# krm01/Snappy.jl

Hardware: AMD Instinct MI355X
Metric: GB/s compressed+decompressed (batched blocks) at 1/2/4/8 GPUs; % HBM peak (higher is better)
Workload: dtype u8; 1 GPU; configs 2+3: 10000 x 64 KiB text blocks per GPU, fast-mode compress + uncompress round trip per step; blocks_per_gpu=10000, block_bytes=65536, parallelism=dp1 (blocks sharded per rank, RCCL size all-gather)

## Files before the change

### snappy.jl_amd/csrc/sm_dec_walk.h

```cpp
#pragma once
#include "sm_device.h"

namespace sm {

typedef uint16_t __attribute__((aligned(1))) du16u;
typedef uint32_t __attribute__((aligned(1))) du32u;
typedef uint64_t __attribute__((aligned(1))) du64u;

constexpr uint32_t kMaxBatchLit = 200;
constexpr int kWalkLevels = 5;
constexpr int kJtRow = 256;
constexpr int kJt = kWalkLevels * kJtRow / 2;
__device__ inline uint32_t load_word(const uint8_t* __restrict__ in, uint32_t N, uint32_t p) {
  if (p + 3 < N && (((uintptr_t)(in + p)) & 3) == 0) return *reinterpret_cast<const uint32_t*>(in + p);
  uint32_t v = 0;
#pragma unroll
  for (int k = 0; k < 4; ++k) v |= (p + k < N ? (uint32_t)in[p + k] : 0u) << (8 * k);
  return v;
}

__device__ inline uint64_t load8z(const uint8_t* __restrict__ in, uint32_t N, uint32_t p) {
  return (uint64_t)load_word(in, N, p) | ((uint64_t)load_word(in, N, p + 4) << 32);
}

__device__ inline uint32_t pack_sizes(uint32_t cur, uint32_t nxt) {
  const uint32_t K = cur & 0x03030303u, H = (cur >> 2) & 0x3f3f3f3fu;
  const uint32_t csz = __builtin_amdgcn_perm(0u, 0x05030200u, K);
  const uint32_t ml = __builtin_amdgcn_perm(0u, 0x000000ffu, K);
  uint32_t sz = (csz & ~ml) | ((H + 0x02020202u) & ml);
  const uint32_t h60 = (H + 0x44444444u) & 0x80808080u & ml;
  if (h60) {
    const uint32_t hm = h60 | (h60 - (h60 >> 7));
    const uint32_t b = __builtin_amdgcn_alignbyte(nxt, cur, 1);
    const uint32_t e = cur ^ 0xf0f0f0f0u;
    const uint32_t ne = (((e & 0x7f7f7f7fu) + 0x7f7f7f7fu) | e) & 0x80808080u;
    const uint32_t bb = (((b >> 1) & 0x7f7f7f7fu) + 0x1c1c1c1cu) & 0x80808080u;
    const uint32_t st = ne | bb;
    const uint32_t sm = st | (st - (st >> 7));
    const uint32_t v = (b | sm) + (0x03030303u & ~sm);
    sz = (sz & ~hm) | (v & hm);
  }
  return sz;
}

__device__ inline bool walk_stop_literal(uint32_t c, uint64_t lit) {
  return (c & 3) == 0 && ((c >> 2) >= 61 || lit > kMaxBatchLit);
}

__device__ inline uint32_t walk_window(uint64_t cw, uint32_t rlim, uint16_t* jt16, uint32_t lane, uint32_t& cpos,
                                       uint32_t& csz, uint32_t& sizes) {
  uint8_t* const jt = reinterpret_cast<uint8_t*>(jt16);
  rlim = min(rlim, 255u);
  sizes = pack_sizes((uint32_t)cw, (uint32_t)(cw >> 32));
  auto rd = [&](int k, uint32_t x) -> uint32_t { return jt[k * kJtRow + x]; };
  auto row = [&](int k, const uint32_t (&J)[4]) {
    *reinterpret_cast<uint32_t*>(jt + k * kJtRow + 4 * lane) = J[0] | (J[1] << 8) | (J[2] << 16) | (J[3] << 24);
  };
  uint32_t J[4];
#pragma unroll
  for (int j = 0; j < 4; ++j) {
    const uint32_t p = 4 * lane + j;
    const uint32_t sz = (sizes >> (8 * j)) & 0xff;
    J[j] = sz == 255 ? p : min(p + sz, 255u);
  }
  row(0, J);
  uint32_t c = 0;
#pragma unroll
  for (int k = 1; k < kWalkLevels; ++k) {
    __atomic_signal_fence(__ATOMIC_SEQ_CST);
    const uint32_t t = rd(k - 1, c);
#pragma unroll
    for (int j = 0; j < 4; ++j) J[j] = rd(k - 1, J[j]);
    c = ((lane >> (k - 1)) & 1u) ? t : c;
    row(k, J);
  }
  __atomic_signal_fence(__ATOMIC_SEQ_CST);
  {
    const uint32_t t = rd(kWalkLevels - 1, c);
    c = ((lane >> (kWalkLevels - 1)) & 1u) ? t : c;
  }
  if (lane >= 32) {
    c = rd(kWalkLevels - 1, c);
    c = rd(kWalkLevels - 1, c);
  }
  const uint32_t szw = __shfl(sizes, (c >> 2) & 63u, 64);
  const uint32_t sz = (szw >> (8 * (c & 3))) & 0xffu;
  cpos = c;
  csz = sz;
  __atomic_signal_fence(__ATOMIC_SEQ_CST);
  return (uint32_t)__builtin_popcountll(ballot(c < rlim && sz != 255));
}

__device__ inline void stage_bytes(uint8_t* buf, const uint8_t* __restrict__ in, uint32_t N, uint32_t s, uint32_t len,
                                   uint32_t lane) {
  constexpr int kU = 6;
  uint32_t* dst = reinterpret_cast<uint32_t*>(buf);
  const uint32_t nw = (len + 3) / 4;
  if (N == 0) {
    for (uint32_t k = lane; k < nw; k += kWave) dst[k] = 0;
    return;
  }
  const uint32_t mis = (uint32_t)((uintptr_t)(in + s) & 3u);
  const uint32_t* src = reinterpret_cast<const uint32_t*>(in + s - mis);
  const int64_t klast = ((intptr_t)((uintptr_t)(in + N - 1) & ~(uintptr_t)3) - (intptr_t)src) / 4;
  for (uint32_t k0 = lane; k0 < nw; k0 += kU * kWave) {
    uint32_t w[kU];
#pragma unroll
    for (int u = 0; u < kU; ++u) {
      const int64_t k = k0 + u * kWave;
      w[u] = __builtin_amdgcn_alignbyte(src[min(k + 1, klast)], src[min(k, klast)], mis);
    }
#pragma unroll
    for (int u = 0; u < kU; ++u) {
      const uint64_t b = (uint64_t)s + 4 * (k0 + u * kWave);
      const uint64_t v = b < N ? (uint64_t)N - b : 0u;
      w[u] &= v >= 4 ? 0xffffffffu : (uint32_t)((1ull << (8 * v)) - 1);
    }
#pragma unroll
    for (int u = 0; u < kU; ++u)
      if (k0 + u * kWave < nw) dst[k0 + u * kWave] = w[u];
  }
}

__device__ inline Tag tag_at(const uint8_t* buf, uint32_t rel) { return decode_tag8(lds_ld64(buf, rel)); }

__device__ inline uint32_t window_tags(const uint8_t* buf, uint32_t rel0, uint32_t rlim, uint16_t* jt, uint32_t lane,
                                       uint32_t& rel, uint32_t& next, uint32_t& outb, uint32_t& excl) {
  uint32_t cpos, csz, sizes;
  const uint32_t ntok = walk_window(lds_ld64(buf, rel0 + 4 * lane), rlim, jt, lane, cpos, csz, sizes);
  const bool mine = lane < ntok;
  const uint32_t c = buf[rel0 + (mine ? cpos : 0u)];
  outb = !mine ? 0u : window_out_bytes(c, csz);
  excl = scan_dpp(outb) - outb;
  rel = rel0 + cpos;
  next = rel + csz;
  return ntok;
}

__device__ inline int32_t parse_header(const uint8_t* in, uint32_t N, uint32_t lane, uint32_t& size, uint32_t& ip) {
  const uint32_t hb = (lane < 5 && lane < N) ? in[lane] : 0;
  return smc::parse_varint32([&](uint32_t i) { return readlane(hb, i); }, N, size, ip);
}

}
```

### snappy.jl_amd/csrc/sm_decompress.hip

```cpp
#include "sm_dec_walk.h"
#include "sm_internal.h"

namespace sm {

constexpr uint32_t kRing = 1024;
constexpr uint32_t kRingMirror = 96;


__device__ inline void ring_put(uint8_t* ring, uint32_t base, uint32_t word, uint32_t lane) {
  uint32_t r = base & (kRing - 1);
  reinterpret_cast<uint32_t*>(ring + r)[lane] = word;
  if (r == 0 && lane < kRingMirror / 4) reinterpret_cast<uint32_t*>(ring + kRing)[lane] = word;
}

__device__ inline uint64_t ring_get8(const uint8_t* ring, uint32_t pos) { return lds_ld64(ring, pos & (kRing - 1)); }

__device__ inline void ring_fill(const uint8_t* __restrict__ in, uint32_t N, uint32_t wb, uint8_t* ring, uint32_t& pre1,
                                 uint32_t& pre2, uint32_t lane) {
  uint32_t w[5];
  if ((((uintptr_t)(in + wb)) & 3) == 0 && wb + 1280 <= N) {
    const uint32_t* s = reinterpret_cast<const uint32_t*>(in + wb) + lane;
#pragma unroll
    for (int i = 0; i < 5; ++i) w[i] = s[64 * i];
  } else {
#pragma unroll
    for (int i = 0; i < 5; ++i) w[i] = load_word(in, N, wb + 256 * i + 4 * lane);
  }
  ring_put(ring, wb, w[0], lane);
  ring_put(ring, wb + 256, w[1], lane);
  ring_put(ring, wb + 512, w[2], lane);
  pre1 = w[3];
  pre2 = w[4];
}

#ifndef SM_DEC_WIN
#define SM_DEC_WIN 2560
#endif
constexpr uint32_t kWin = SM_DEC_WIN;
#ifndef SM_DEC_BOUT
#define SM_DEC_BOUT 512
#endif
constexpr uint32_t kBatchOut = SM_DEC_BOUT;
#ifndef SM_DEC_KEEP
#define SM_DEC_KEEP 480
#endif
constexpr uint32_t kKeep = SM_DEC_KEEP;
constexpr uint32_t kWinPad = 16;
static_assert(kKeep + 15 + kBatchOut + 32 <= kWin && kKeep >= 80 && kWin % 16 == 0, "window bounds");
static_assert(kKeep + 15 <= 16 * kWave, "win_shift moves at most one 16-byte unit per lane");

typedef __attribute__((address_space(3))) uint32_t lds_u32;

__device__ inline uint4 lds_get16(uint32_t a, uint32_t k) {
  const lds_u32* w = (const lds_u32*)(size_t)((a & ~3u) + k);
  const uint32_t w0 = w[0], w1 = w[1], w2 = w[2], w3 = w[3], w4 = w[4];
  return make_uint4(__builtin_amdgcn_alignbyte(w1, w0, a), __builtin_amdgcn_alignbyte(w2, w1, a),
                    __builtin_amdgcn_alignbyte(w3, w2, a), __builtin_amdgcn_alignbyte(w4, w3, a));
}

__device__ inline uint4 trim16(uint4 v, uint32_t len) {
  uint32_t l8 = len << 3;
  asm("" : "+v"(l8));
  uint64_t mlo, mhi;
  asm("v_lshrrev_b64 %0, %1, -1" : "=v"(mlo) : "v"(64 - min(l8, 64u)));
  asm("v_lshrrev_b64 %0, %1, -1" : "=v"(mhi) : "v"(128 - l8));
  const bool hi = len > 8;
  return make_uint4(v.x & (uint32_t)mlo, v.y & (uint32_t)(mlo >> 32), hi ? v.z & (uint32_t)mhi : 0u,
                    hi ? v.w & (uint32_t)(mhi >> 32) : 0u);
}

__device__ inline void lds_or16(uint32_t a, uint32_t k, uint4 v) {
  const uint32_t wa = ((a - 1u) & ~3u) + k, t = 0u - a;
  const uint32_t u0 = __builtin_amdgcn_alignbyte(v.x, 0u, t);
  const uint32_t u1 = __builtin_amdgcn_alignbyte(v.y, v.x, t);
  const uint32_t u2 = __builtin_amdgcn_alignbyte(v.z, v.y, t);
  const uint32_t u3 = __builtin_amdgcn_alignbyte(v.w, v.z, t);
  const uint32_t u4 = __builtin_amdgcn_alignbyte(0u, v.w, t);
  asm volatile("ds_or_b32 %0, %1\nds_or_b32 %0, %2 offset:4\nds_or_b32 %0, %3 offset:8\nds_or_b32 %0, %4 offset:12\n"
               "ds_or_b32 %0, %5 offset:16"
               : : "v"(wa), "v"(u0), "v"(u1), "v"(u2), "v"(u3), "v"(u4) : "memory");
}

__device__ inline void win_init(uint8_t* win, uint32_t lane) {
  for (uint32_t u = lane; u < kWin / 16; u += kWave) reinterpret_cast<uint4*>(win)[u] = make_uint4(0, 0, 0, 0);
}

__device__ inline void win_shift(uint8_t* win, uint32_t& wbase, uint32_t op, uint32_t lane) {
  const uint32_t nb = (op - kKeep) & ~15u;
  const uint32_t d = nb - wbase, n = (op - nb + 15) >> 4;
  uint4* w = reinterpret_cast<uint4*>(win);
  uint4 v = make_uint4(0, 0, 0, 0);
  if (lane < n) v = w[(d >> 4) + lane];
  __atomic_signal_fence(__ATOMIC_SEQ_CST);
  for (uint32_t u = lane; u < kWin / 16; u += kWave) w[u] = u < n ? v : make_uint4(0, 0, 0, 0);
  wbase = nb;
}

__device__ inline void win_flush(uint8_t* out, const uint8_t* win, uint32_t wbase, uint32_t from, uint32_t to,
                                 uint32_t lane) {
  if (to <= from) return;
  const uint32_t h = min((16u - (from & 15u)) & 15u, to - from);
  if (lane < h) out[from + lane] = win[from + lane - wbase];
  from += h;
  const uint32_t nb = (to - from) >> 4;
  for (uint32_t k = lane; k < nb; k += kWave) {
    const uint32_t x = from + 16 * k;
    const uint4 v = *reinterpret_cast<const uint4*>(win + (x - wbase));
    *reinterpret_cast<du64u*>(out + x) = ((uint64_t)v.y << 32) | v.x;
    *reinterpret_cast<du64u*>(out + x + 8) = ((uint64_t)v.w << 32) | v.z;
  }
  from += nb << 4;
  if (lane < to - from) out[from + lane] = win[from + lane - wbase];
}

template <uint32_t kLit = 4, bool kWhole = false>
__device__ int32_t decode_stream_batch(const uint8_t* __restrict__ in, uint32_t N, uint32_t ip, uint32_t ip_end,
                                       uint32_t size, uint8_t* out, uint32_t op0, uint32_t frag_lo, uint8_t* ring,
                                       uint16_t* jt, uint8_t* win, uint32_t lane, uint32_t& op_end,
                                       uint32_t op_lim = 0xffffffffu) {
  if (kWhole) {
    ip_end = N;
    frag_lo = 0;
    op_lim = 0xffffffffu;
  }
  uint32_t wb = ip & ~255u;
  uint32_t pre1, pre2;
  ring_fill(in, N, wb, ring, pre1, pre2, lane);
  bool issue_pre2 = false;
  uint32_t op = op0, flushed = op0;
  const uint32_t wlo = op0 & ~15u;
  uint32_t wbase = wlo;
  win_init(win, lane);
  const uint32_t winA = lds_addr(win), ringA = lds_addr(ring);
  const bool in_al = (((uintptr_t)in) & 3) == 0;
  const int64_t Nm1 = min((int64_t)N - 1, (int64_t)ip_end);

  uint32_t guard = N + 1;
  const bool narrow = N < 0x80000000u && size <= 0xffff0000u;
  while ((int64_t)ip < Nm1 && (kWhole || op < op_lim)) {
    if (__builtin_expect(--guard == 0, 0)) return kErrDevice;
    if (ip >= wb + 256) {
      if (__builtin_expect(ip < wb + 512, 1)) {
        ring_put(ring, wb + 768, pre1, lane);
        pre1 = pre2;
        wb += 256;
        issue_pre2 = true;
      } else {
        wb = ip & ~255u;
        ring_fill(in, N, wb, ring, pre1, pre2, lane);
        issue_pre2 = false;
      }
    }
    const uint32_t wlim = (int64_t)(ip + 256) < Nm1 ? ip + 256 : (uint32_t)Nm1;
    uint32_t cpos, csz, sizes;
    const uint32_t ntok = walk_window(ring_get8(ring, ip + 4 * lane), wlim - ip, jt, lane, cpos, csz, sizes);
    uint32_t tpos = 0, ipw = ip, tnext = 0;
    bool big = false;
    if (__builtin_expect(ntok != 0, 1)) {
      tpos = ip + cpos;
      tnext = cpos + csz;
      ipw = ip + readlane(tnext, ntok - 1);
    }
    if (ipw < wlim) {
      const uint32_t rel = ipw - ip;
      big = ((readlane(sizes, rel >> 2) >> ((rel & 3) * 8)) & 0xff) == 255;
    }

    if (__builtin_expect(ntok != 0, 1)) {
      const bool mine = lane < ntok;
      const uint64_t hv = ring_get8(ring, mine ? tpos : wb);
      const uint32_t c = (uint32_t)hv & 0xff;
      const uint32_t kind = c & 3, hi = c >> 2;
      const bool iscopy = kind != 0, k1 = kind == 1;
      const uint32_t len = k1 ? 4 + (hi & 7) : hi + 1;
      const uint32_t offhi = k1 ? (c << 3) & 0x700u : 0u;
      const uint32_t tl = (c + 16) >> 8;
      const uint32_t tr_raw = (uint32_t)(hv >> 8);
      uint64_t hm;
      asm("v_lshlrev_b64 %0, %1, -1" : "=v"(hm) : "v"(8 * csz - 8));
      const uint32_t offset = offhi + (tr_raw & ~(uint32_t)hm);
      const uint32_t litlen = csz - 1 - tl;
      const uint32_t olen = mine ? (iscopy ? len : litlen) : 0u;
      const uint32_t incl = scan_dpp(olen);
      const uint32_t opt = op + incl - olen;
      const uint32_t lsrc = tpos + 1 + tl;
      const uint64_t minem = ntok == 64 ? ~0ull : ((1ull << ntok) - 1);
      const uint64_t copya = ballot(iscopy) & minem;

      const uint32_t X_all = readlane(incl, ntok - 1);
      const bool clean = narrow && op <= size && op + X_all <= size && ipw <= N;
      uint64_t badm = ballot(opt <= offset - 1u);
      if (!kWhole) badm |= ballot(opt - offset < frag_lo);
      if (__builtin_expect(!clean || (badm & copya) != 0, 0)) {
        const int64_t avail_out = (int64_t)size - (int64_t)opt;
        const int64_t avail_in = (int64_t)N - (int64_t)lsrc;
        const bool e_off = (int64_t)opt <= (int64_t)(uint32_t)(offset - 1u);
        const bool e_cross = !kWhole && opt - offset < frag_lo;
        const bool e_len = !((len <= 16) & (offset >= 8) & (avail_out >= 16)) & (avail_out < (int64_t)len);
        const bool e_lit = (avail_out < (int64_t)litlen) | (avail_in < (int64_t)litlen);
        const int32_t ec = e_off ? kErrCopyOffset : (e_cross ? kErrCross : (e_len ? kErrCopyLength : kOk));
        const int32_t err = !mine ? kOk : (iscopy ? ec : (e_lit ? kErrLiteral : kOk));
        const uint64_t em = ballot(err != kOk);
        if (em != 0) return (int32_t)readlane((uint32_t)err, ctz64(em));
      }
      uint32_t nt = ntok;
      if (__builtin_expect(X_all > kBatchOut || (!kWhole && readlane(opt, ntok - 1) >= op_lim), 0)) {
        nt = (uint32_t)__builtin_popcountll(ballot(mine && incl <= kBatchOut && (kWhole || opt < op_lim)));
        ipw = ip + readlane(tnext, nt - 1);
        big = false;
      }
      const uint32_t X = readlane(incl, nt - 1);

      if (op - wbase + X + 32 > kWin) win_shift(win, wbase, op, lane);
      const uint32_t O0 = op;
      const uint32_t slo = opt - offset;
      const uint32_t shi = slo + min(len, offset);
      const uint64_t all = nt == 64 ? ~0ull : ((1ull << nt) - 1);
      const uint64_t copym = copya & all;
      const uint64_t longm = ballot(litlen > 64) & ~copym & all;
      const uint64_t gm = ballot(slo < wbase) & copym;
      const bool gsrc = inverse_ballot(gm);
      uint64_t done = longm | ~all;
      if (gm) __threadfence_block();

      uint64_t lm = longm;
      while (lm) {
        const uint32_t t = ctz64(lm);
        lm &= lm - 1;
        const uint32_t o = readlane(opt, t), sr = readlane(lsrc, t), L = readlane(litlen, t);
        const uint32_t k = 16 * lane;
        if (k < L) lds_or16(winA + (o - wbase) + k, 0, trim16(lds_get16(ringA + ((sr + k) & (kRing - 1)), 0), min(16u, L - k)));
      }

      if (__builtin_expect(done != ~0ull, 1)) {
        const uint64_t rm = ~done & (~copym | (ballot(shi <= O0) & ballot(offset >= 16)));
        const uint32_t L = iscopy ? len : litlen;
        const uint32_t sa = iscopy ? winA + (slo - wbase) : ringA + (lsrc & (kRing - 1));
        const uint32_t da = winA + (opt - wbase);
        const uint8_t* gs = out + slo;
#pragma unroll
        for (uint32_t base = 0; base < 64; base += 16) {
          const uint64_t am = rm & ballot(L > base);
          if (!am) break;
          if (inverse_ballot(am)) {
            uint4 v;
            if (gsrc) {
              const du64u* g = reinterpret_cast<const du64u*>(gs + base);
              const uint64_t a = g[0], b = g[1];
              v = make_uint4((uint32_t)a, (uint32_t)(a >> 32), (uint32_t)b, (uint32_t)(b >> 32));
            } else {
              v = lds_get16(sa, base);
            }
            lds_or16(da, base, trim16(v, min(L - base, 16u)));
          }
        }
        done |= rm;
      }
      __atomic_signal_fence(__ATOMIC_SEQ_CST);
      uint64_t rest = ~done;
      while (rest) {
        const uint32_t t = ctz64(rest);
        rest &= rest - 1;
        const uint32_t o = readlane(opt, t), sl = readlane(slo, t), L = readlane(len, t), off = readlane(offset, t);
        if (lane < L) {
          uint32_t k = lane;
          if (k >= off) {
            const uint32_t q = (uint32_t)(((float)k + 0.5f) * __builtin_amdgcn_rcpf((float)off));
            k -= q * off;
          }
          win[o + lane - wbase] = win[sl + k - wbase];
        }
        __atomic_signal_fence(__ATOMIC_SEQ_CST);
      }
      op += X;
      if (!kWhole && __builtin_expect(op > op_lim, 0)) return kErrCross;
      win_flush(out, win, wbase, flushed, op & ~15u, lane);
      flushed = max(flushed, op & ~15u);
      ip = ipw;
    }
    if (issue_pre2) {
      pre2 = (in_al && wb + 1280 <= N) ? reinterpret_cast<const uint32_t*>(in + wb + 1024)[lane]
                                       : load_word(in, N, wb + 1024 + 4 * lane);
      issue_pre2 = false;
    }

    if (__builtin_expect(big && (kWhole || op < op_lim), 0)) {
      const uint64_t hv = ring_get8(ring, ip);
      const Tag t = with_trailer(tag_head(uniform((uint32_t)hv & 0xff)), uniform((uint32_t)(hv >> 8)));
      const uint32_t litlen = t.literal_len();
      const uint32_t lsrc = ip + 1 + t.taglen;
      const int64_t avail_out = (int64_t)size - (int64_t)op;
      const int64_t avail_in = (int64_t)N - (int64_t)lsrc;
      if (avail_out < (int64_t)litlen || avail_in < (int64_t)litlen) return kErrLiteral;
      if (!kWhole && (uint64_t)op + litlen > op_lim) return kErrCross;
      if (litlen <= kMaxBatchLit) {
        if (op - wbase + litlen + 32 > kWin) win_shift(win, wbase, op, lane);
        const uint32_t k = 16 * lane;
        if (k < litlen)
          lds_or16(winA + (op - wbase) + k, 0, trim16(lds_get16(ringA + ((lsrc + k) & (kRing - 1)), 0), min(16u, litlen - k)));
        __atomic_signal_fence(__ATOMIC_SEQ_CST);
        op += litlen;
        win_flush(out, win, wbase, flushed, op & ~15u, lane);
        flushed = max(flushed, op & ~15u);
        ip = lsrc + litlen;
        continue;
      }
      win_flush(out, win, wbase, flushed, op, lane);
      const uint8_t* s = in + lsrc;
      uint32_t head = (uint32_t)((16 - ((uintptr_t)s & 15)) & 15);
      if (head > litlen) head = litlen;
      if (lane < head) out[op + lane] = s[lane];
      const uint4* s16 = reinterpret_cast<const uint4*>(s + head);
      const uint32_t n16 = (litlen - head) >> 4;
      uint8_t* d = out + op + head;
      uint32_t k = lane;
      for (; k + (kLit - 1) * kWave < n16; k += kLit * kWave) {
        uint4 v[kLit];
#pragma unroll
        for (uint32_t j = 0; j < kLit; ++j) v[j] = s16[k + j * kWave];
#pragma unroll
        for (uint32_t j = 0; j < kLit; ++j) {
          *reinterpret_cast<du64u*>(d + 16 * (k + j * kWave)) = ((uint64_t)v[j].y << 32) | v[j].x;
          *reinterpret_cast<du64u*>(d + 16 * (k + j * kWave) + 8) = ((uint64_t)v[j].w << 32) | v[j].z;
        }
      }
      for (; k < n16; k += kWave) {
        uint4 v0 = s16[k];
        *reinterpret_cast<du64u*>(d + 16 * k) = ((uint64_t)v0.y << 32) | v0.x;
        *reinterpret_cast<du64u*>(d + 16 * k + 8) = ((uint64_t)v0.w << 32) | v0.z;
      }
      const uint32_t done16 = head + (n16 << 4);
      if (lane < litlen - done16) out[op + done16 + lane] = s[done16 + lane];
      const uint32_t opn = op + litlen;
      const uint32_t nb = (opn - min(opn - wlo, kKeep)) & ~15u;
      const uint32_t nk = opn - nb;
      __threadfence_block();
      const uint8_t* q = out + nb;
      for (uint32_t u = lane; u < kWin / 16; u += kWave) {
        const uint32_t x = 16 * u;
        uint4 v = make_uint4(0, 0, 0, 0);
        if (x + 16 <= nk) {
          const du64u* g = reinterpret_cast<const du64u*>(q + x);
          const uint64_t a = g[0], b = g[1];
          v = make_uint4((uint32_t)a, (uint32_t)(a >> 32), (uint32_t)b, (uint32_t)(b >> 32));
        } else if (x < nk) {
          uint64_t lo = 0, hi = 0;
          for (uint32_t i = 0; i < nk - x; ++i) {
            const uint64_t bt = (uint64_t)q[x + i] << (8 * (i & 7));
            if (i < 8) lo |= bt;
            else hi |= bt;
          }
          v = make_uint4((uint32_t)lo, (uint32_t)(lo >> 32), (uint32_t)hi, (uint32_t)(hi >> 32));
        }
        reinterpret_cast<uint4*>(win)[u] = v;
      }
      wbase = nb;
      op += litlen;
      flushed = op;
      ip = lsrc + litlen;
    }
  }
  win_flush(out, win, wbase, flushed, op, lane);
  op_end = op;
  return kOk;
}

#ifndef SM_DEC_OCC
#define SM_DEC_OCC 7
#endif
template <uint32_t kLit = 4>
__device__ inline void decompress_block(const DecompressArgs& a, uint32_t b, uint8_t* sring, uint16_t* sjt, uint8_t* swin,
                                        uint32_t lane) {
  const uint8_t* in = a.one_n ? a.in : a.in + a.in_off[b];
  const uint32_t N = a.one_n ? a.one_n : a.in_len[b];
  uint8_t* dst = a.one_n ? a.out : a.out + a.out_off[b];
  const uint32_t cap = a.one_n ? a.one_cap : a.out_cap[b];

  uint32_t size = cap, ip = 0;
  if (N >= kOutLenError) {
    if (lane == 0) {
      a.status[b] = kErrDevice;
      a.out_len[b] = 0;
    }
    return;
  }
  int32_t st = a.raw ? kOk : parse_header(in, N, lane, size, ip);
  if (st == kOk && size > cap) st = kBufferTooSmall;
  if (st == kOk) {
    uint32_t op_end = 0;
    st = decode_stream_batch<kLit, true>(in, N, ip, N, size, dst, 0, 0, sring, sjt, swin, lane, op_end);
    if (st == kOk && op_end != size) st = kErrInvalid;
  }
  if (lane == 0) {
    a.status[b] = st;
    a.out_len[b] = st == kOk ? size : 0;
  }
}

__global__ __launch_bounds__(64, SM_DEC_OCC) void k_decompress(DecompressArgs a) {
  __shared__ __attribute__((aligned(16))) uint8_t sring[kRing + kRingMirror];
  __shared__ __attribute__((aligned(16))) uint16_t sjt[kJt];
  __shared__ __attribute__((aligned(16))) uint8_t swin[kWinPad + kWin];
  decompress_block(a, blockIdx.x, sring, sjt, swin + kWinPad, lane_id());
}

__global__ __launch_bounds__(64, 1) void k_decompress_one(DecompressArgs a) {
  __shared__ __attribute__((aligned(16))) uint8_t sring[kRing + kRingMirror];
  __shared__ __attribute__((aligned(16))) uint16_t sjt[kJt];
  __shared__ __attribute__((aligned(16))) uint8_t swin[kWinPad + kWin];
  decompress_block<16>(a, 0, sring, sjt, swin + kWinPad, lane_id());
}

__global__ __launch_bounds__(64, 4) void k_decompress_frags(const uint8_t* __restrict__ in, uint32_t N, uint32_t size,
                                                            uint8_t* out, const StreamFrag* frags, int32_t* status) {
  __shared__ __attribute__((aligned(16))) uint8_t sring[kRing + kRingMirror];
  __shared__ __attribute__((aligned(16))) uint16_t sjt[kJt];
  __shared__ __attribute__((aligned(16))) uint8_t swin[kWinPad + kWin];
  __shared__ __attribute__((aligned(16))) uint8_t sbuf[kIdxChunk + kIdxPad];
  const uint32_t f = blockIdx.x, lane = lane_id();
  const StreamFrag fr = frags[f];
  stage_bytes(sbuf, in, N, fr.y, kIdxChunk + kIdxPad, lane);
  __syncthreads();
  uint64_t p = fr.y, o = fr.O;
  int32_t st = kOk;
  while (o < fr.F) {
    const uint32_t rel0 = (uint32_t)(p - fr.y);
    if (rel0 >= kIdxChunk + 16) {
      st = kErrCross;
      break;
    }
    uint32_t rel, next, ob, excl;
    const uint32_t ntok = window_tags(sbuf, rel0, min(kIdxChunk + 16 - rel0, 256u), sjt, lane, rel, next, ob, excl);
    if (ntok == 0) {
      const Tag t = tag_at(sbuf, rel0);
      o += t.out_bytes();
      p += t.size();
      continue;
    }
    const uint64_t hit = ballot(lane < ntok && o + excl >= fr.F);
    if (hit) {
      const uint32_t t = ctz64(hit);
      o += readlane(excl, t);
      p = fr.y + readlane(rel, t);
      break;
    }
    o += readlane(excl + ob, ntok - 1);
    p = fr.y + readlane(next, ntok - 1);
  }
  if (st == kOk && o != fr.F) st = kErrCross;
  if (st == kOk) {
    uint32_t op_end = 0;
    st = decode_stream_batch(in, N, (uint32_t)p, N, size, out, fr.F, fr.F, sring, sjt, swin + kWinPad, lane, op_end, fr.lim);
    if (st == kOk && op_end != (fr.lim == 0xffffffffu ? size : fr.lim)) st = kErrCross;
  }
  if (lane == 0) status[f] = st;
}

__global__ __launch_bounds__(64) void k_validate(const uint8_t* __restrict__ d_in, const uint64_t* in_off,
                                                 const uint32_t* in_len, int32_t* status) {
  __shared__ __attribute__((aligned(16))) uint8_t buf[320];
  __shared__ __attribute__((aligned(16))) uint16_t jt[kJt];
  const uint32_t b = blockIdx.x, lane = lane_id();
  const uint8_t* in = d_in + in_off[b];
  const uint32_t N = in_len[b];
  if (N >= kOutLenError) {
    if (lane == 0) status[b] = kErrDevice;
    return;
  }
  uint32_t size, ip;
  int32_t st = parse_header(in, N, lane, size, ip);
  uint64_t op = 0, p = ip;
  const uint64_t lim = N ? N - 1 : 0;
  while (st == kOk && p < lim) {
    stage_bytes(buf, in, N, (uint32_t)p, 320, lane);
    __atomic_signal_fence(__ATOMIC_SEQ_CST);
    uint32_t rel, next, ob, excl;
    const uint32_t ntok = window_tags(buf, 0, (uint32_t)min(lim - p, (uint64_t)256), jt, lane, rel, next, ob, excl);
    const bool mine = lane < ntok || (ntok == 0 && lane == 0);
    const Tag t = tag_at(buf, mine ? rel : 0u);
    const uint32_t taglen = t.taglen, litlen = t.literal_len();
    const uint64_t opt = op + (ntok ? excl : 0u);
    const int32_t err = mine ? check_tag(t, opt, size, p + (ntok ? rel : 0u) + 1 + taglen, N) : kOk;
    const uint64_t em = ballot(err != kOk);
    if (em) {
      st = (int32_t)readlane((uint32_t)err, ctz64(em));
      break;
    }
    if (ntok == 0) {
      op += readlane(litlen, 0);
      p += 1 + readlane(taglen, 0) + (uint64_t)readlane(litlen, 0);
    } else {
      op += readlane(excl + ob, ntok - 1);
      p += readlane(next, ntok - 1);
    }
  }
  if (st == kOk && op != size) st = kErrInvalid;
  if (lane == 0) status[b] = st;
}

__global__ __launch_bounds__(256) void k_uncompressed_length(const uint8_t* __restrict__ d_in, const uint64_t* in_off,
                                                             const uint32_t* in_len, uint32_t nblk, uint32_t* out_len,
                                                             int32_t* status) {
  const uint32_t b = blockIdx.x * blockDim.x + threadIdx.x;
  if (b >= nblk) return;
  const uint8_t* in = d_in + in_off[b];
  const uint32_t N = in_len[b];
  uint32_t v = 0, hv;
  int32_t st = kErrDevice;
  if (N < kOutLenError) st = smc::parse_varint32([&](uint32_t i) { return (uint32_t)in[i]; }, N, v, hv);
  out_len[b] = st == kOk ? v : 0;
  status[b] = st;
}

hipError_t launch_validate(const uint8_t* in, const uint64_t* in_off, const uint32_t* in_len, uint32_t nblk,
                           int32_t* status, hipStream_t s) {
  if (nblk == 0) return hipSuccess;
  hipLaunchKernelGGL(k_validate, dim3(nblk), dim3(64), 0, s, in, in_off, in_len, status);
  return hipGetLastError();
}

hipError_t launch_uncompressed_length(const uint8_t* in, const uint64_t* in_off, const uint32_t* in_len,
                                      uint32_t nblk, uint32_t* out_len, int32_t* status, hipStream_t s) {
  if (nblk == 0) return hipSuccess;
  hipLaunchKernelGGL(k_uncompressed_length, dim3((nblk + 255) / 256), dim3(256), 0, s, in, in_off, in_len, nblk,
                     out_len, status);
  return hipGetLastError();
}

hipError_t launch_decompress_frags(const uint8_t* in, uint32_t N, uint32_t size, uint8_t* out,
                                   const StreamFrag* frags, uint32_t nfrag, int32_t* status, hipStream_t s) {
  if (nfrag == 0) return hipSuccess;
  hipLaunchKernelGGL(k_decompress_frags, dim3(nfrag), dim3(64), 0, s, in, N, size, out, frags, status);
  return hipGetLastError();
}

hipError_t launch_decompress(const DecompressArgs& a, int , hipStream_t s) {
  if (a.nblk == 0) return hipSuccess;
  if (a.one_n && a.nblk == 1)
    hipLaunchKernelGGL(k_decompress_one, dim3(1), dim3(64), 0, s, a);
  else
    hipLaunchKernelGGL(k_decompress, dim3(a.nblk), dim3(64), 0, s, a);
  return hipGetLastError();
}

}
```

Measured before the change: 402.7 GB/s.

## Overlap next window tag walk with current batch copies in decompressor

The decompress loop now runs the next window's tag walk (and the ring advance and prefetch) before the current batch's LDS and global copies, so the walk's LDS latency chain overlaps the copy work. The first global-source 16-byte load is also issued earlier, and paired 8-byte unaligned global stores and loads become single unaligned 16-byte vector accesses. This adds carried state across iterations (walked flag, saved walk results) and raises register pressure. The early walk is skipped near limits or on big literals.

```diff
diff --git a/snappy.jl_amd/csrc/sm_dec_walk.h b/snappy.jl_amd/csrc/sm_dec_walk.h
--- a/snappy.jl_amd/csrc/sm_dec_walk.h
+++ b/snappy.jl_amd/csrc/sm_dec_walk.h
@@ -6,6 +6,17 @@
 typedef uint16_t __attribute__((aligned(1))) du16u;
 typedef uint32_t __attribute__((aligned(1))) du32u;
 typedef uint64_t __attribute__((aligned(1))) du64u;
+typedef uint32_t __attribute__((ext_vector_type(4), aligned(1))) du128u;
+
+__device__ inline uint4 ld16u(const uint8_t* p) {
+  const du128u v = *reinterpret_cast<const du128u*>(p);
+  return make_uint4(v.x, v.y, v.z, v.w);
+}
+__device__ inline void st16u(uint8_t* p, uint4 v) {
+  du128u t;
+  t.x = v.x, t.y = v.y, t.z = v.z, t.w = v.w;
+  *reinterpret_cast<du128u*>(p) = t;
+}
 
 constexpr uint32_t kMaxBatchLit = 200;
 constexpr int kWalkLevels = 5;
diff --git a/snappy.jl_amd/csrc/sm_decompress.hip b/snappy.jl_amd/csrc/sm_decompress.hip
--- a/snappy.jl_amd/csrc/sm_decompress.hip
+++ b/snappy.jl_amd/csrc/sm_decompress.hip
@@ -105,9 +105,7 @@
   const uint32_t nb = (to - from) >> 4;
   for (uint32_t k = lane; k < nb; k += kWave) {
     const uint32_t x = from + 16 * k;
-    const uint4 v = *reinterpret_cast<const uint4*>(win + (x - wbase));
-    *reinterpret_cast<du64u*>(out + x) = ((uint64_t)v.y << 32) | v.x;
-    *reinterpret_cast<du64u*>(out + x + 8) = ((uint64_t)v.w << 32) | v.z;
+    st16u(out + x, *reinterpret_cast<const uint4*>(win + (x - wbase)));
   }
   from += nb << 4;
   if (lane < to - from) out[from + lane] = win[from + lane - wbase];
@@ -133,27 +131,40 @@
   win_init(win, lane);
   const uint32_t winA = lds_addr(win), ringA = lds_addr(ring);
   const bool in_al = (((uintptr_t)in) & 3) == 0;
-  const int64_t Nm1 = min((int64_t)N - 1, (int64_t)ip_end);
+  const uint32_t Nm1 = min(N ? N - 1 : 0u, ip_end);
 
   uint32_t guard = N + 1;
   const bool narrow = N < 0x80000000u && size <= 0xffff0000u;
-  while ((int64_t)ip < Nm1 && (kWhole || op < op_lim)) {
+  auto ring_advance = [&]() {
+    ring_put(ring, wb + 768, pre1, lane);
+    pre1 = pre2;
+    asm volatile("" : "+v"(pre1));
+    wb += 256;
+    issue_pre2 = true;
+  };
+  auto fetch_pre2 = [&]() {
+    pre2 = (in_al && wb + 1280 <= N) ? reinterpret_cast<const uint32_t*>(in + wb + 1024)[lane]
+                                     : load_word(in, N, wb + 1024 + 4 * lane);
+    issue_pre2 = false;
+  };
+  bool walked = false;
+  uint32_t ntok = 0, cpos = 0, csz = 0, sizes = 0;
+  while (ip < Nm1 && (kWhole || op < op_lim)) {
     if (__builtin_expect(--guard == 0, 0)) return kErrDevice;
-    if (ip >= wb + 256) {
-      if (__builtin_expect(ip < wb + 512, 1)) {
-        ring_put(ring, wb + 768, pre1, lane);
-        pre1 = pre2;
-        wb += 256;
-        issue_pre2 = true;
-      } else {
-        wb = ip & ~255u;
-        ring_fill(in, N, wb, ring, pre1, pre2, lane);
-        issue_pre2 = false;
-      }
-    }
-    const uint32_t wlim = (int64_t)(ip + 256) < Nm1 ? ip + 256 : (uint32_t)Nm1;
-    uint32_t cpos, csz, sizes;
-    const uint32_t ntok = walk_window(ring_get8(ring, ip + 4 * lane), wlim - ip, jt, lane, cpos, csz, sizes);
+    const uint32_t wlim = ip + 256 < Nm1 ? ip + 256 : Nm1;
+    if (!walked) {
+      if (ip >= wb + 256) {
+        if (__builtin_expect(ip < wb + 512, 1)) {
+          ring_advance();
+        } else {
+          wb = ip & ~255u;
+          ring_fill(in, N, wb, ring, pre1, pre2, lane);
+          issue_pre2 = false;
+        }
+      }
+      ntok = walk_window(ring_get8(ring, ip + 4 * lane), wlim - ip, jt, lane, cpos, csz, sizes);
+    }
+    walked = false;
     uint32_t tpos = 0, ipw = ip, tnext = 0;
     bool big = false;
     if (__builtin_expect(ntok != 0, 1)) {
@@ -219,9 +230,23 @@
       const uint64_t copym = copya & all;
       const uint64_t longm = ballot(litlen > 64) & ~copym & all;
       const uint64_t gm = ballot(slo < wbase) & copym;
-      const bool gsrc = inverse_ballot(gm);
       uint64_t done = longm | ~all;
+      const uint64_t rm = ~done & (~copym | (ballot(shi <= O0) & ballot(offset >= 16)));
+      const uint64_t fm = gm & rm;
+      const uint32_t L = iscopy ? len : litlen;
+      const uint32_t da = winA + (opt - wbase);
+      const uint8_t* gs = out + slo;
+
+      const bool early = !big && ipw < Nm1 && (kWhole || O0 + X < op_lim) && ipw < wb + 512;
+      if (issue_pre2) fetch_pre2();
+      if (early && ipw >= wb + 256) {
+        ring_advance();
+        fetch_pre2();
+      }
+
       if (gm) __threadfence_block();
+      uint4 fv = make_uint4(0, 0, 0, 0);
+      if (inverse_ballot(fm)) fv = ld16u(gs);
 
       uint64_t lm = longm;
       while (lm) {
@@ -232,30 +257,27 @@
         if (k < L) lds_or16(winA + (o - wbase) + k, 0, trim16(lds_get16(ringA + ((sr + k) & (kRing - 1)), 0), min(16u, L - k)));
       }
 
-      if (__builtin_expect(done != ~0ull, 1)) {
-        const uint64_t rm = ~done & (~copym | (ballot(shi <= O0) & ballot(offset >= 16)));
-        const uint32_t L = iscopy ? len : litlen;
+      if (__builtin_expect(early, 1)) {
+        const uint32_t wl2 = ipw + 256 < Nm1 ? ipw + 256 : Nm1;
+        ntok = walk_window(ring_get8(ring, ipw + 4 * lane), wl2 - ipw, jt, lane, cpos, csz, sizes);
+        walked = true;
+      }
+      if (__builtin_expect(rm != 0, 1)) {
+        const bool gsrc = inverse_ballot(fm);
         const uint32_t sa = iscopy ? winA + (slo - wbase) : ringA + (lsrc & (kRing - 1));
-        const uint32_t da = winA + (opt - wbase);
-        const uint8_t* gs = out + slo;
 #pragma unroll
         for (uint32_t base = 0; base < 64; base += 16) {
           const uint64_t am = rm & ballot(L > base);
           if (!am) break;
           if (inverse_ballot(am)) {
             uint4 v;
-            if (gsrc) {
-              const du64u* g = reinterpret_cast<const du64u*>(gs + base);
-              const uint64_t a = g[0], b = g[1];
-              v = make_uint4((uint32_t)a, (uint32_t)(a >> 32), (uint32_t)b, (uint32_t)(b >> 32));
-            } else {
-              v = lds_get16(sa, base);
-            }
+            if (gsrc) v = base == 0 ? fv : ld16u(gs + base);
+            else v = lds_get16(sa, base);
             lds_or16(da, base, trim16(v, min(L - base, 16u)));
           }
         }
-        done |= rm;
-      }
+      }
+      done |= rm;
       __atomic_signal_fence(__ATOMIC_SEQ_CST);
       uint64_t rest = ~done;
       while (rest) {
@@ -278,11 +300,7 @@
       flushed = max(flushed, op & ~15u);
       ip = ipw;
     }
-    if (issue_pre2) {
-      pre2 = (in_al && wb + 1280 <= N) ? reinterpret_cast<const uint32_t*>(in + wb + 1024)[lane]
-                                       : load_word(in, N, wb + 1024 + 4 * lane);
-      issue_pre2 = false;
-    }
+    if (issue_pre2) fetch_pre2();
 
     if (__builtin_expect(big && (kWhole || op < op_lim), 0)) {
       const uint64_t hv = ring_get8(ring, ip);
@@ -319,16 +337,9 @@
 #pragma unroll
         for (uint32_t j = 0; j < kLit; ++j) v[j] = s16[k + j * kWave];
 #pragma unroll
-        for (uint32_t j = 0; j < kLit; ++j) {
-          *reinterpret_cast<du64u*>(d + 16 * (k + j * kWave)) = ((uint64_t)v[j].y << 32) | v[j].x;
-          *reinterpret_cast<du64u*>(d + 16 * (k + j * kWave) + 8) = ((uint64_t)v[j].w << 32) | v[j].z;
-        }
-      }
-      for (; k < n16; k += kWave) {
-        uint4 v0 = s16[k];
-        *reinterpret_cast<du64u*>(d + 16 * k) = ((uint64_t)v0.y << 32) | v0.x;
-        *reinterpret_cast<du64u*>(d + 16 * k + 8) = ((uint64_t)v0.w << 32) | v0.z;
-      }
+        for (uint32_t j = 0; j < kLit; ++j) st16u(d + 16 * (k + j * kWave), v[j]);
+      }
+      for (; k < n16; k += kWave) st16u(d + 16 * k, s16[k]);
       const uint32_t done16 = head + (n16 << 4);
       if (lane < litlen - done16) out[op + done16 + lane] = s[done16 + lane];
       const uint32_t opn = op + litlen;
```

Result: faster. 411.2 GB/s (median of 6 runs) (+2.1%).
